# edantec/MPC_benchmark

Measured on AMD Instinct MI355X. Metric: mpc_solves_per_sec, higher is better.
Workload: dtype f64

## Files before the change

### mpc_benchmark_amd/csrc/legs.h

```cpp
#pragma once
#include "mfma_blocks.h"
#include "solver_kernels.h"

#define LEG_BARRIER() asm volatile("s_waitcnt lgkmcnt(0)\n\ts_barrier" ::: "memory")

#define LEG_LAUNDER() do { asm volatile("" : "+v"(tid), "+v"(lane)); wv = __builtin_amdgcn_readfirstlane(tid >> 6); } while (0)

#define LK_THREADS 512
#define LK_U 20
#define LK_PT 13
#define LK_TILES 5

struct LkLds {
  int np, mp, nzp, lda, ldp, ldm, nb, nbm;
  int AB, PR, TM, ZN, vec, total_bytes;
  unsigned mg_nzp, mg_np, mg_mp;
};
static inline constexpr LkLds make_lk_lds(int n, int m) {
  LkLds s{};
  s.np = (n + 15) & ~15; s.mp = (m + 15) & ~15; s.nzp = s.np + s.mp; s.lda = s.nzp + 1; s.ldp = s.np + 1; s.ldm = s.mp + 1;
  s.nb = s.np / 16; s.nbm = s.mp / 16;
  s.mg_nzp = magic_div(s.nzp); s.mg_np = magic_div(s.np); s.mg_mp = magic_div(s.mp);
  int o = 0;
  auto take = [&](int cnt) { int r = o; o += (cnt + 1) & ~1; return r; };
  const int pr = s.np * s.ldp > s.mp * s.np + s.mp * s.ldm ? s.np * s.ldp : s.mp * s.np + s.mp * s.ldm;
  s.AB = take(s.np * s.lda); s.PR = take(pr); s.TM = take(6 * s.nzp + 6 * s.np + 40); s.ZN = take(16 * s.ldm); s.vec = take(s.mp + 3 * s.np + 80 + 8);
  s.total_bytes = o * 8;
  return s;
}

template <int MP, int FN = 0, int FM = 0>
__global__ void __launch_bounds__(LK_THREADS) k_leg_knot(SolverArgs a, LkLds Srt, int chunk) {
  constexpr bool FX = FN > 0;
  constexpr LkLds SC_ = FX ? make_lk_lds(FN, FM) : LkLds{};
  LkLds S_ = Srt;
  if constexpr (FX) S_ = SC_;
  const LkLds& S = S_;
  constexpr int NAB = (80 * (80 + MP) + LK_THREADS - 1) / LK_THREADS, NK = (MP * 80 + LK_THREADS - 1) / LK_THREADS;
  constexpr int NMU = (MP * MP + LK_THREADS - 1) / LK_THREADS, NZN = (16 * MP + LK_THREADS - 1) / LK_THREADS;
  const Layout& L = a.L;
  const int b = blockIdx.y;
  int tid = threadIdx.x, lane = tid & 63;
  constexpr int nthr = LK_THREADS, nw = LK_THREADS / 64;
  int wv = __builtin_amdgcn_readfirstlane(tid >> 6);
  const InstState& st = a.inst[b];
  if (st.done || st.skip_step) return;
  const int n = FX ? FN : L.n, nz = FX ? FN + FM : L.nz, np = S.np, mp = S.mp, nzp = S.nzp, lda = S.lda, ldp = S.ldp, ldm = S.ldm, nb = S.nb, nbm = S.nbm;
  const int kbeg = blockIdx.x * chunk, kend = (kbeg + chunk < L.N) ? kbeg + chunk : L.N;
  const double mud = st.mu * a.opt.dyn_al_scale;
  extern __shared__ __attribute__((aligned(16))) double sm[];
  double *AB = sm + S.AB, *PR = sm + S.PR, *ZN = sm + S.ZN, *vec = sm + S.vec;
  double *KM = PR, *PT = PR, *U1 = PR, *MU = PR + mp * np;
  double *TMP = sm + S.TM, *PT6 = TMP + 6 * nzp, *c6 = PT6 + 6 * np;
  double *kf = vec, *y0 = vec + mp, *z0 = y0 + np, *t6 = z0 + np, *g6 = t6 + 36, *mxs = g6 + 36;
  int* cnt = (int*)(mxs + np);
  long long tk0_ = clock64();
#define LK_PROF(slot) do { if (a.prof && k == 1 && b == 1 && tid == 0) { const long long t1_ = clock64(); a.prof[64 + 32 + (slot)] += (double)(t1_ - tk0_); tk0_ = t1_; } } while (0)

  double pab[NAB], pkm[NK], ptv[LK_PT], pmu[NMU], pzn[NZN], psm = 0.0, pact = 0.0;
  auto request_ab = [&](int k) {
    const double* kn = knot_ptr(a, b, k);
    const double* g = gain_ptr(a, b, k);
    const int m = (int)kn[L.oMISC + MISC_M], c = (int)kn[L.oMISC + MISC_NC];
#pragma unroll
    for (int u = 0; u < NAB; ++u) {
      const int idx = tid + u * nthr, i = qdiv(idx, S.mg_nzp), zp = (idx - qdiv(idx, S.mg_nzp) * nzp);
      const int z = (zp < n) ? zp : ((zp >= np && zp - np < m) ? n + zp - np : -1);
      pab[u] = (idx < np * nzp && i < n && z >= 0) ? kn[L.oAB + (size_t)i * nz + z] : 0.0;
    }
#pragma unroll
    for (int u = 0; u < NK; ++u) {
      const int idx = tid + u * nthr, l = qdiv(idx, S.mg_np), j = (idx - qdiv(idx, S.mg_np) * np);
      pkm[u] = (idx < mp * np && l < m && j < n) ? g[L.oK + l * n + j] : 0.0;
    }
    psm = (tid < mp) ? ((tid < m) ? g[L.ok + tid] : 0.0) : ((tid >= 64 && tid < 100) ? g[L.oT6 + tid - 64] : ((tid >= 128 && tid < 128 + n) ? g[L.omx + tid - 128] : 0.0));
    pact = (tid < c) ? kn[L.oACT + tid] : 0.0;
  };
  auto request_pt = [&](int k) {
    const double* g = gain_ptr(a, b, k);
#pragma unroll
    for (int u = 0; u < LK_PT; ++u) {
      const int idx = tid + u * nthr, i = qdiv(idx, S.mg_np), j = (idx - qdiv(idx, S.mg_np) * np);
      ptv[u] = (idx < np * np && i < n && j < n) ? g[L.oMx + i * n + j] : 0.0;
    }
  };
  auto request_mu = [&](int k) {
    const double* g = gain_ptr(a, b, k);
#pragma unroll
    for (int u = 0; u < NMU; ++u) { const int idx = tid + u * nthr; pmu[u] = (idx < mp * mp) ? g[L.oMu + idx] : 0.0; }
#pragma unroll
// ... 160 lines not shown
            if (row < m && col < n) g[L.oKu + row * n + col] = -ures[sidx][q];
          }
        }
      }
#ifdef LK_SUBPROF
      LK_PROF(9);
#endif
      LEG_BARRIER();
      LK_PROF(5);
      for (int t = wv; t < nb * nb; t += nw) {
        const int ri = t / nb, cj = t % nb, col = cj * 16 + (lane & 15);
        double ptt[4];
#pragma unroll
        for (int q = 0; q < 4; ++q) {
          const int row = ri * 16 + (lane >> 4) + 4 * q;
          const bool in = row < n && col < n;
          ptt[q] = (in && row >= 6 && col >= 6) ? g[L.oMx + row * n + col] : 0.0;
        }
        d4_t acc = d4_t{0, 0, 0, 0};
        mma_tile<false>(acc, AB + (ri * 16) * lda + np, lda, 1, U1 + cj * 16, np, 1, mp, lane);
#pragma unroll
        for (int q = 0; q < 4; ++q) {
          const int row = ri * 16 + (lane >> 4) + 4 * q;
          if (row < n && col < n) {
            const double tt = (row < 6 && col < 6) ? g6[row * 6 + col] : (row == col ? 1.0 : 0.0);
            const double tp = (row < 6 && col < 6) ? c6[row * 6 + col] : (col < 6 ? PT6[row * 6 + col] : (row < 6 ? PT6[col * 6 + row] : ptt[q]));
            g[L.oGam + row * n + col] = -acc[q] - mud * (tt - mud * tp);
          }
        }
      }
      LK_PROF(6);
    } else if (par_next) request_mu(k + 1);
  }
}

struct LcLds { int np, ldp, nb; int LM, BA, BB, vec, total_bytes; unsigned mg_np, mg_ldp; };
static inline constexpr int lc_ld(int np) { int ld = np; while ((ld & 31) != 16) ++ld; return ld; }
static inline constexpr LcLds make_lc_lds(int n) {
  LcLds s{};
  s.np = (n + 15) & ~15; s.ldp = lc_ld(s.np); s.nb = s.np / 16;
  s.mg_np = magic_div(s.np); s.mg_ldp = magic_div(s.ldp);
  int o = 0;
  auto take = [&](int cnt) { int r = o; o += (cnt + 1) & ~1; return r; };
  s.LM = take(s.np * s.ldp); s.BA = take(s.np * s.ldp); s.BB = take(s.np * s.ldp); s.vec = take(3 * s.np + 16);
  s.total_bytes = o * 8;
  return s;
}
#define LC_TILES 4
#define LC_STILES 2

template <int FN = 0>
__global__ void __launch_bounds__(LK_THREADS) k_leg_condense(SolverArgs a, LcLds Srt) {
  constexpr bool FX = FN > 0;
  constexpr LcLds SC_ = FX ? make_lc_lds(FN) : LcLds{};
  LcLds S_ = Srt;
  if constexpr (FX) S_ = SC_;
  const LcLds& S = S_;
  const Layout& L = a.L;
  constexpr int nthr = LK_THREADS, nw = LK_THREADS / 64;
  const int j = blockIdx.x, b = blockIdx.y;
  int tid = threadIdx.x, lane = tid & 63, wv = __builtin_amdgcn_readfirstlane(tid >> 6);
  const InstState& st = a.inst[b];
  if (st.done || st.skip_step) return;
  const int n = FX ? FN : L.n, np = S.np, ldp = S.ldp, nb = S.nb;
  const int ks = leg_start(a, j), ke = leg_start(a, j + 1) - 1;
  extern __shared__ __attribute__((aligned(16))) double sm[];
  double *LM = sm + S.LM, *BA = sm + S.BA, *BB = sm + S.BB, *sg = sm + S.vec, *phi = sg + np;
  for (int idx = tid; idx < np * ldp; idx += nthr) { const int i = qdiv(idx, S.mg_ldp), c0 = (idx - qdiv(idx, S.mg_ldp) * ldp); LM[idx] = (i == c0 && i < n) ? 1.0 : 0.0; }
  for (int i = tid; i < np; i += nthr) sg[i] = 0.0;
  d4_t sacc[LC_STILES];
  int tri[LC_STILES], tcj[LC_STILES];
#pragma unroll
  for (int sidx = 0; sidx < LC_STILES; ++sidx) {
    sacc[sidx] = d4_t{0, 0, 0, 0};
    int ri = 0, rem = wv + sidx * nw;
    while (rem > ri) { rem -= ri + 1; ++ri; }
    tri[sidx] = ri; tcj[sidx] = rem;
  }
  const int nst = nb * (nb + 1) / 2;
  double pa[LK_PT], pb[LK_PT], pphi;
  auto prefetch = [&](int kk) {
    const double* gk = gain_ptr(a, b, kk);
#pragma unroll
    for (int u = 0; u < LK_PT; ++u) {
      const int idx = tid + u * nthr, i = qdiv(idx, S.mg_np), c0 = (idx - qdiv(idx, S.mg_np) * np);
      const bool ok = idx < np * np && i < n && c0 < n;
      const int src = ok ? i * n + c0 : 0;
      pa[u] = gk[L.oPhi + src] * (ok ? 1.0 : 0.0);
      pb[u] = gk[L.oGam + src] * (ok ? 1.0 : 0.0);
    }
    pphi = gk[L.ophi + (tid < n ? tid : 0)];
  };
  prefetch(ke);
// ... 48 lines not shown
    LC_PROF(5);
    LEG_BARRIER();
    LC_PROF(6);
    LEG_LAUNDER();
    double* gk = gain_ptr(a, b, k);
#pragma unroll
    for (int sidx = 0; sidx < LC_TILES; ++sidx) {
      const int t = wv + sidx * nw;
      if (t < nb * nb) {
        const int ri = t / nb, cj = t % nb, col = cj * 16 + (lane & 15);
        tile_store(LM + (ri * 16) * ldp + cj * 16, ldp, lres[sidx], lane);
#pragma unroll
        for (int q = 0; q < 4; ++q) { const int row = ri * 16 + (lane >> 4) + 4 * q; if (row < n && col < n) gk[L.oLm + row * n + col] = lres[sidx][q]; }
      }
    }
    LEG_BARRIER();
    LC_PROF(7);
  }
  double* lr = leg_ptr(a, b, j);
#pragma unroll
  for (int sidx = 0; sidx < LC_STILES; ++sidx)
    if (wv + sidx * nw < nst) {
      const int col = tcj[sidx] * 16 + (lane & 15);
#pragma unroll
      for (int q = 0; q < 4; ++q) {
        const int row = tri[sidx] * 16 + (lane >> 4) + 4 * q;
        if (row < n && col < n) {
          if (tri[sidx] != tcj[sidx]) { lr[L.lSg + row * n + col] = sacc[sidx][q]; lr[L.lSg + col * n + row] = sacc[sidx][q]; }
          else if (col <= row) { lr[L.lSg + row * n + col] = sacc[sidx][q]; lr[L.lSg + col * n + row] = sacc[sidx][q]; }
        }
      }
    }
  for (int i = tid; i < n; i += nthr) lr[L.lsg + i] = sg[i];
}

struct LxLds { int np, mp, ldp, nb, nbm; int PC, MA, RB, vec, iw, total_bytes; unsigned mg_np, mg_ldp; };
static inline constexpr LxLds make_lx_lds(int n, int m) {
  LxLds s{};
  s.np = (n + 15) & ~15; s.mp = (m + 15) & ~15; s.ldp = s.np + 1; s.nb = s.np / 16; s.nbm = s.mp / 16;
  s.mg_np = magic_div(s.np); s.mg_ldp = magic_div(s.ldp);
  int o = 0;
  auto take = [&](int cnt) { int r = o; o += (cnt + 1) & ~1; return r; };
  s.PC = take(s.np * s.ldp); s.MA = take(s.np * s.ldp); s.RB = take(s.np * s.ldp);
  s.vec = take(8 * s.np + 16 + 128);
  s.iw = o;
  s.total_bytes = o * 8 + (2 * s.np + 8) * 4;
  return s;
}

template <bool TR>
DEV void leg_load_mat(double* dst, int ldp, int np, const double* src, int n, int tid, int nthr, unsigned mg_np) {
  const struct { unsigned mg_np; } S = {mg_np};
  double v[LK_PT];
#pragma unroll
  for (int u = 0; u < LK_PT; ++u) {
    const int idx = tid + u * nthr, i = qdiv(idx, S.mg_np), c0 = (idx - qdiv(idx, S.mg_np) * np);
    const bool ok = idx < np * np && i < n && c0 < n;
    v[u] = src[ok ? i * n + c0 : 0] * (ok ? 1.0 : 0.0);
  }
#pragma unroll
  for (int u = 0; u < LK_PT; ++u) {
    const int idx = tid + u * nthr, i = qdiv(idx, S.mg_np), c0 = (idx - qdiv(idx, S.mg_np) * np);
    if (idx < np * np) dst[TR ? c0 * ldp + i : i * ldp + c0] = v[u];
  }
}

// ... 380 lines not shown
```

### mpc_benchmark_amd/csrc/mpc_hip.hip

```cpp
#include <hip/hip_runtime.h>
#include <mutex>
#include <map>
#include <cmath>
#include <cstdio>
#include <cstdlib>
#include <cstring>
#include <limits>
#include <stdexcept>
#include <string>
#include <utility>
#include <vector>

#include "eval_multibody_host.h"
#include "eval_reuse_kernels.h"
#include "eval_vector.h"
#include "riccati_mfma.h"
#include "closed_loop.h"
#include "legs.h"
#include "legs_tree.h"
#include "pipeline_glue.h"
#include "pipeline_ikid_glue.h"
#include "pipeline_contacts.h"
#include "pipeline_fd_glue.h"
#include "sim_record.h"
// ... 122 lines not shown
  bool refine_now = false;
  SimPlant plant;
  std::vector<uint8_t> slot_dirty;
  bool dirty_all = false;
  bool spec_skip_pass = false;
  unsigned long long dirty_now[MPC_DIRTY_WORDS] = {};
  static constexpr int PATCH_RING = 4;
  char* patch_pin[PATCH_RING] = {};
  size_t patch_cap[PATCH_RING] = {};
  hipEvent_t patch_ev[PATCH_RING] = {};
  int patch_next = 0;
  char* d_patch = nullptr;
  size_t d_patch_cap = 0;
  double* h_xnext[2] = {nullptr, nullptr};
  std::vector<double> leg_mu;
  static constexpr int ASYNC_DEPTH = 2;
  InstState* h_status[ASYNC_DEPTH] = {nullptr, nullptr};
  hipEvent_t status_ev[ASYNC_DEPTH] = {nullptr, nullptr};
  int async_head = 0, async_pending = 0;
  static constexpr int STAGE_RING = 8;
  char* stage_pin[STAGE_RING] = {};
  hipEvent_t stage_ev[STAGE_RING] = {};
  int stage_next = 0;
  RicLds ric{};
  int ric_fixed = 0;
  ClLds cl{};
  bool use_mfma_riccati = false;
  LkLds lk{};
  LcLds lc{};
  LxLds lx{};
  bool legs_ok = false;
  bool env_chain = false, env_plain = false, env_reject_failed = false;
  int env_tree_sweeps = 0, env_trace = -1;
  double* d_legbuf = nullptr;
  double* d_treebuf = nullptr;
  int leg_cap = 0;
  TreeDesc tree{};
  bool use_tree() const {
    return eff_legs() >= 3 && d_treebuf != nullptr && !env_chain;
  }
  bool leg_guess_valid = false;
  int leg_guess_now = 0;
  int eff_legs() const {
    if (!legs_ok) return 1;
    int J = opt.riccati_legs;
    if (J > MPC_MAX_LEGS) J = MPC_MAX_LEGS;
    if (J > L.N) J = L.N;
    return J < 1 ? 1 : J;
  }
  struct ProfSlot {
    const char* name;
    std::vector<std::pair<hipEvent_t, hipEvent_t>> ev;
    size_t used = 0;
  };
  bool profiling = false;
  unsigned prof_mask = ~0u;
  std::vector<ProfSlot> prof;

  template <class F> void timed(int slot, const char* name, F&& launch) {
    if (!profiling || !((prof_mask >> slot) & 1u) || pass_is_corrector) { launch(); return; }
    if ((int)prof.size() <= slot) prof.resize(slot + 1);
    ProfSlot& p = prof[slot];
    p.name = name;
    if (p.used == p.ev.size()) {
      hipEvent_t e0, e1;
      HIP_OK(hipEventCreate(&e0));
// ... 47 lines not shown
  HIP_OK(hipStreamSynchronize(s->stream));
}

static void ensure_leg_capacity(mpc_solver* s, int legs) {
  const Layout& L = s->L;
  int need = legs < 1 ? 1 : legs;
  if (need >= 3 && need < 4) need = 4;
  if (need <= s->leg_cap) return;
  HIP_OK(hipStreamSynchronize(s->stream));
  auto regrow = [&](double*& p, size_t count) {
    if (p) HIP_OK(hipFree(p));
    p = nullptr;
    HIP_OK(hipMalloc((void**)&p, (count ? count : 1) * sizeof(double)));
    HIP_OK(hipMemsetAsync(p, 0, (count ? count : 1) * sizeof(double), s->stream));
  };
  const size_t B = L.B;
  regrow(s->d_work, B * need * (size_t)L.work_stride);
  if (s->legs_ok) {
    regrow(s->d_legbuf, B * (size_t)(need > 1 ? need - 1 : 1) * L.leg_stride);
    regrow(s->d_treebuf, B * (size_t)need * L.tree_stride);
  }
  s->leg_cap = need;
  s->leg_guess_valid = false;
  HIP_OK(hipStreamSynchronize(s->stream));
}

static void create_impl(mpc_solver* s, const mpc_dims& d) {
  s->dims = d;
  { const char* e;
    e = getenv("MPC_LEGS_CHAIN"); s->env_chain = e && atoi(e) > 0;
    e = getenv("MPC_LEGS_PLAIN"); s->env_plain = e && atoi(e) > 0;
    e = getenv("MPC_HIP_REJECT_FAILED"); s->env_reject_failed = e && atoi(e) > 0;
    e = getenv("MPC_TREE_SWEEPS"); s->env_tree_sweeps = e ? atoi(e) : 0;
    e = getenv("MPC_HIP_TRACE"); s->env_trace = e ? atoi(e) : -1; }
  HIP_OK(hipSetDevice(d.device));
  {
    static int created = 0;
    const char* pe = getenv("MPC_HIP_STREAM_PRIO");
    if (pe && atoi(pe) > 0) {
      int lo = 0, hi = 0;
      HIP_OK(hipDeviceGetStreamPriorityRange(&lo, &hi));
      const int levels = lo - hi + 1;
      const int prio = hi + (created++ % levels);
      HIP_OK(hipStreamCreateWithPriority(&s->stream, hipStreamNonBlocking, prio));
      if (atoi(pe) > 1) fprintf(stderr, "[mpc] stream priority %d (range %d..%d)\n", prio, hi, lo);
    } else {
      HIP_OK(hipStreamCreateWithFlags(&s->stream, hipStreamNonBlocking));
    }
  }
  Layout& L = s->L;
  L.N = d.horizon; L.B = d.batch; L.space = d.space; L.nx = d.nx; L.n = d.ndx; L.m = d.nu; L.c = d.nc_max > 0 ? d.nc_max : 1;
  L.nj = 0;
  L.max_stage_ints = d.max_stage_ints; L.max_stage_doubles = d.max_stage_doubles;
  L.n_alpha = 8;
  make_layout(L);
  Layout& T = s->LT;
  T = L;
  {
    int o = 0;
    auto take = [&](int cnt) { int r = o; o += align2(cnt); return r; };
    T.oCV = take(L.c); T.oCT = take(L.c); T.oLO = take(L.c); T.oHI = take(L.c); T.oDT = take(L.c); T.oACT = take(L.c);
    T.oF = take(L.n); T.oMISC = take(MISC_COUNT);
    T.oH = T.oG = T.oAB = T.oE6 = T.oT6k = T.oD12 = T.oCD = T.oXD = T.oWR = T.oXN = 0;
    T.knot_stride = o;
  }
  if (s->riccati_lds() > 160 * 1024) throw std::runtime_error("problem dimensions exceed the LDS budget of the Riccati kernel");
  const size_t B = d.batch, N1 = d.horizon + 1, N = d.horizon;
  s->d_stage_desc = s->alloc<int32_t>(N1 * L.max_stage_ints);
// ... 32 lines not shown
    if (c3.total_bytes > 160 * 1024) c3 = make_ric_lds(L.n, L.m, L.c, 3, 0);
    if (c3.total_bytes <= 160 * 1024 && c3.ovl && (c3.st_lds || c3.mp * c3.np <= L.n * L.nz)) s->ric = c3;
  }
  if (s->ric.total_bytes > 160 * 1024 && ((L.n + 15) & ~15) * ((L.m + 15) & ~15) <= L.n * L.n) {
    s->ric = make_ric_lds(L.n, L.m, L.c, 2);
    if (s->ric.total_bytes > 160 * 1024) s->ric = make_ric_lds(L.n, L.m, L.c, 2, 0);
  }
  if (s->ric.total_bytes > 160 * 1024) s->ric = make_ric_lds(L.n, L.m, L.c, 0);
  if (s->ric.total_bytes > 160 * 1024) s->ric = make_ric_lds(L.n, L.m, L.c, 0, 0);
  if (sq_ok && s->ric.gfull) { s->ric.sq = 1; s->ric.nv = L.n / 2; }
  s->cl = make_cl_lds(L.n, L.m);
  if (s->cl.total_bytes <= 160 * 1024)
    lds_attr_max((const void*)k_closed_loop, s->cl.total_bytes);
  s->use_mfma_riccati = s->ric.total_bytes <= 160 * 1024 && (s->ric.st_lds || s->ric.mp * s->ric.np <= L.n * L.nz) && !getenv("MPC_HIP_GENERIC_RICCATI");
  if (s->use_mfma_riccati)
  {
    lds_attr_max((const void*)k_riccati_mfma<RIC_THREADS, 96>, s->ric.total_bytes);
    lds_attr_max((const void*)k_riccati_mfma<RIC_THREADS, 80>, s->ric.total_bytes);
    lds_attr_max((const void*)k_riccati_mfma<RIC_THREADS, 96, true>, s->ric.total_bytes);
    lds_attr_max((const void*)k_riccati_mfma<RIC_THREADS, 80, true>, s->ric.total_bytes);
    lds_attr_max((const void*)k_riccati_mfma<RIC_SMALL_THREADS, 16>, s->ric.total_bytes);
  }
  s->lk = make_lk_lds(L.n, L.m); s->lc = make_lc_lds(L.n); s->lx = make_lx_lds(L.n, L.m);
  s->legs_ok = s->use_mfma_riccati && s->ric.np <= 80 && s->ric.mp <= 48 && L.c <= 256 && s->ric.gfull >= 1 && s->lk.total_bytes <= 160 * 1024 &&
               s->lc.total_bytes <= 160 * 1024 && s->lx.total_bytes <= 160 * 1024 && !getenv("MPC_HIP_NO_LEGS");
  if (s->legs_ok) {
    lds_attr_max((const void*)k_riccati_mfma<RIC_THREADS, 80, true, true>, s->ric.total_bytes);
    s->ric_fixed = 0;
    if (!getenv("MPC_HIP_GENERIC_DIMS") && s->ric.sq) {
#define X(ID, FN, FM, GF, ST, NPV, MPV) if (!s->ric_fixed && L.n == FN && L.m == FM && L.nz == FN + FM && ric_same_layout(s->ric, ric_fixed_layout(FN, FM, true, GF, ST))) s->ric_fixed = ID;
      MPC_FIXED_MODELS(X)
#undef X
    }
#define X(ID, FN, FM, GF, ST, NPV, MPV) if (s->ric_fixed == ID) { \
      lds_attr_max((const void*)k_riccati_mfma<RIC_THREADS, 80, true, true, FN, FM, GF, ST>, s->ric.total_bytes); \
      lds_attr_max((const void*)k_leg_knot<MPV, FN, FM>, s->lk.total_bytes); \
      lds_attr_max((const void*)k_leg_condense<FN>, s->lc.total_bytes); \
      lds_attr_max((const void*)k_leg_compose<NPV, FN, FM>, s->lx.total_bytes); \
      lds_attr_max((const void*)k_leg_tree_down<NPV, FN, FM>, s->lx.total_bytes); }
    MPC_FIXED_MODELS(X)
#undef X
    lds_attr_max((const void*)k_riccati_mfma<RIC_THREADS, 80, false, true>, s->ric.total_bytes);
    lds_attr_max((const void*)k_riccati_mfma<RIC_SMALL_THREADS, 16, false, true>, s->ric.total_bytes);
    lds_attr_max((const void*)k_leg_knot<16>, s->lk.total_bytes);
    lds_attr_max((const void*)k_leg_knot<32>, s->lk.total_bytes);
    lds_attr_max((const void*)k_leg_knot<48>, s->lk.total_bytes);
    lds_attr_max((const void*)k_leg_condense<0>, s->lc.total_bytes);
    lds_attr_max((const void*)k_leg_consensus<16>, s->lx.total_bytes);
    lds_attr_max((const void*)k_leg_consensus<32>, s->lx.total_bytes);
    lds_attr_max((const void*)k_leg_consensus<48>, s->lx.total_bytes);
    lds_attr_max((const void*)k_leg_consensus<64>, s->lx.total_bytes);
    lds_attr_max((const void*)k_leg_consensus<80>, s->lx.total_bytes);
    lds_attr_max((const void*)k_leg_compose<16>, s->lx.total_bytes);
    lds_attr_max((const void*)k_leg_compose<32>, s->lx.total_bytes);
    lds_attr_max((const void*)k_leg_compose<48>, s->lx.total_bytes);
    lds_attr_max((const void*)k_leg_compose<64>, s->lx.total_bytes);
    lds_attr_max((const void*)k_leg_compose<80>, s->lx.total_bytes);
    lds_attr_max((const void*)k_leg_tree_down<16>, s->lx.total_bytes);
    lds_attr_max((const void*)k_leg_tree_down<32>, s->lx.total_bytes);
    lds_attr_max((const void*)k_leg_tree_down<48>, s->lx.total_bytes);
    lds_attr_max((const void*)k_leg_tree_down<64>, s->lx.total_bytes);
    lds_attr_max((const void*)k_leg_tree_down<80>, s->lx.total_bytes);
  }
  ensure_leg_capacity(s, s->eff_legs());
  HIP_OK(hipStreamSynchronize(s->stream));
}

__global__ void __launch_bounds__(256) k_bcast_params(double* inst, const double* shared, int slot, int nslots, int stride) {
  const int b = blockIdx.y;
  const double* src = shared + (size_t)slot * stride;
  double* dst = inst + ((size_t)b * nslots + slot) * stride;
  for (int i = blockIdx.x * 256 + threadIdx.x; i < stride; i += gridDim.x * 256) dst[i] = src[i];
}
static void bcast_slot_to_instances(mpc_solver* s, int slot) {
  if (!s->d_inst_params) return;
  const Layout& L = s->L;
  hipLaunchKernelGGL(k_bcast_params, dim3(4, L.B), dim3(256), 0, s->stream, s->d_inst_params, s->d_stage_params, slot, L.N + 1, L.max_stage_doubles);
  for (int b = 0; b < L.B; ++b)
    std::memcpy(s->h_inst_params.data() + ((size_t)b * (L.N + 1) + slot) * L.max_stage_doubles, s->h_params.data() + (size_t)slot * L.max_stage_doubles,
                (size_t)L.max_stage_doubles * sizeof(double));
// ... 156 lines not shown
  const Layout& L = s->L;
  SolverArgs a = s->args();
  if (ncand <= 0) return;
  if (L.space == MPC_SPACE_VECTOR) {
    if (!trial) hipLaunchKernelGGL(k_eval_vector<0>, dim3(a.only_knot >= 0 ? 1 : L.N + 1, L.B, 1), dim3(64), 0, s->stream, a, s->L, s->d_knots, 0);
    else hipLaunchKernelGGL(k_eval_vector<1>, dim3(L.N + 1, L.B, ncand), dim3(64), 0, s->stream, a, s->LT, s->d_tknots, cand0);
  } else {
    launch_eval_multibody(s->stream, a, s->LT, (trial && !with_derivs) ? s->d_tknots : s->d_knots, s->d_mbwork, s->mb_work_stride, trial, cand0, ncand, 0, 0.0, with_derivs, nullptr, s->contact_dyn);
  }
  HIP_OK(hipGetLastError());
}

static void launch_pass(mpc_solver* s) {
  const Layout& L = s->L;
  if (s->pass_in_run > 0 && s->tick_reuse && s->opt.max_iters <= 4) {
    s->reuse_this_pass = true; s->reuse_same_now = true;
    for (int w = 0; w < MPC_DIRTY_WORDS; ++w) s->dirty_now[w] = 0ull;
  }
  SolverArgs a = s->args();
  if (a.spec_next) hipLaunchKernelGGL(k_copy_spec, dim3(32, L.B), dim3(256), 0, s->stream, a);
  s->timed(0, "k_eval_stage", [&] { launch_eval(s, false); });
  if (a.reuse_on) hipLaunchKernelGGL(k_reproject, dim3(L.N + 1, L.B), dim3(256), 0, s->stream, a);
  s->reuse_this_pass = false; s->reuse_same_now = false;
  s->spec_next_now = false;
  s->timed(1, "k_lagrangian", [&] { hipLaunchKernelGGL(k_lagrangian, dim3(L.N + 1, L.B), dim3(64), 0, s->stream, a); });
  s->timed(2, "k_decide", [&] { hipLaunchKernelGGL(k_decide, dim3(L.B), dim3(128), 0, s->stream, a); });
  a.abdz = nullptr;
  const int J = a.nlegs;
  const bool plain = s->env_plain;
  const bool tree = s->use_tree();
  if (tree && s->tree.J != J) s->tree = make_tree_desc(J);
  int sweeps = (J > 1 && !plain && !s->leg_guess_valid) ? (tree ? s->tree.nlev + 1 : 2) : 1;
  if (tree && !plain && s->env_tree_sweeps > sweeps) sweeps = s->env_tree_sweeps;
  for (int sweep = 0; sweep < sweeps; ++sweep) {
  s->leg_guess_now = (J > 1 && !plain && (s->leg_guess_valid || sweep > 0)) ? 1 : 0;
  a = s->args();
  a.abdz = nullptr;
  s->timed(3, "k_riccati_backward", [&] {
    if (J > 1) {
      if (s->ric.np == 16 && s->ric.mp == 16 && L.c <= RIC_SMALL_THREADS)
        hipLaunchKernelGGL(HIP_KERNEL_NAME(k_riccati_mfma<RIC_SMALL_THREADS, 16, false, true>), dim3(L.B * J), dim3(RIC_SMALL_THREADS), s->ric.total_bytes, s->stream, a, s->ric);
#define X(ID, FN, FM, GF, ST, NPV, MPV) else if (s->ric_fixed == ID) hipLaunchKernelGGL(HIP_KERNEL_NAME(k_riccati_mfma<RIC_THREADS, 80, true, true, FN, FM, GF, ST>), dim3(L.B * J), dim3(RIC_THREADS), s->ric.total_bytes, s->stream, a, s->ric);
      MPC_FIXED_MODELS(X)
#undef X
      else if (s->ric.sq) hipLaunchKernelGGL(HIP_KERNEL_NAME(k_riccati_mfma<RIC_THREADS, 80, true, true>), dim3(L.B * J), dim3(RIC_THREADS), s->ric.total_bytes, s->stream, a, s->ric);
      else hipLaunchKernelGGL(HIP_KERNEL_NAME(k_riccati_mfma<RIC_THREADS, 80, false, true>), dim3(L.B * J), dim3(RIC_THREADS), s->ric.total_bytes, s->stream, a, s->ric);
    }
    else if (s->use_mfma_riccati && s->ric.np == 16 && s->ric.mp == 16 && L.c <= RIC_SMALL_THREADS)
      hipLaunchKernelGGL(HIP_KERNEL_NAME(k_riccati_mfma<RIC_SMALL_THREADS, 16>), dim3(L.B), dim3(RIC_SMALL_THREADS), s->ric.total_bytes, s->stream, a, s->ric);
    else if (s->use_mfma_riccati && s->ric.sq && s->ric.np <= 80) hipLaunchKernelGGL(HIP_KERNEL_NAME(k_riccati_mfma<RIC_THREADS, 80, true>), dim3(L.B), dim3(RIC_THREADS), s->ric.total_bytes, s->stream, a, s->ric);
    else if (s->use_mfma_riccati && s->ric.sq) hipLaunchKernelGGL(HIP_KERNEL_NAME(k_riccati_mfma<RIC_THREADS, 96, true>), dim3(L.B), dim3(RIC_THREADS), s->ric.total_bytes, s->stream, a, s->ric);
    else if (s->use_mfma_riccati && s->ric.np <= 80) hipLaunchKernelGGL(HIP_KERNEL_NAME(k_riccati_mfma<RIC_THREADS, 80>), dim3(L.B), dim3(RIC_THREADS), s->ric.total_bytes, s->stream, a, s->ric);
    else if (s->use_mfma_riccati) hipLaunchKernelGGL(HIP_KERNEL_NAME(k_riccati_mfma<RIC_THREADS, 96>), dim3(L.B), dim3(RIC_THREADS), s->ric.total_bytes, s->stream, a, s->ric);
    else hipLaunchKernelGGL(k_riccati_backward, dim3(L.B), dim3(256), s->riccati_lds(), s->stream, a);
  });
  if (J > 1) {
    s->timed(12, "k_closed_loop", [&] {
      static const int chunk_env = getenv("MPC_LEG_KNOT_CHUNK") ? atoi(getenv("MPC_LEG_KNOT_CHUNK")) : 0;
      const int chunk = chunk_env > 0 ? chunk_env : 1;
      const dim3 grid((L.N + chunk - 1) / chunk, L.B);
      if (false) {}
#define X(ID, FN, FM, GF, ST, NPV, MPV) else if (s->ric_fixed == ID) hipLaunchKernelGGL((k_leg_knot<MPV, FN, FM>), grid, dim3(LK_THREADS), s->lk.total_bytes, s->stream, a, s->lk, chunk);
      MPC_FIXED_MODELS(X)
#undef X
      else if (s->lk.mp <= 16) hipLaunchKernelGGL(k_leg_knot<16>, grid, dim3(LK_THREADS), s->lk.total_bytes, s->stream, a, s->lk, chunk);
      else if (s->lk.mp <= 32) hipLaunchKernelGGL(k_leg_knot<32>, grid, dim3(LK_THREADS), s->lk.total_bytes, s->stream, a, s->lk, chunk);
      else hipLaunchKernelGGL(k_leg_knot<48>, grid, dim3(LK_THREADS), s->lk.total_bytes, s->stream, a, s->lk, chunk);
    });
    s->timed(13, "k_leg_condense", [&] {
      if (false) {}
#define X(ID, FN, FM, GF, ST, NPV, MPV) else if (s->ric_fixed == ID) hipLaunchKernelGGL(k_leg_condense<FN>, dim3(J - 1, L.B), dim3(LK_THREADS), s->lc.total_bytes, s->stream, a, s->lc);
      MPC_FIXED_MODELS(X)
#undef X
      else hipLaunchKernelGGL(k_leg_condense<0>, dim3(J - 1, L.B), dim3(LK_THREADS), s->lc.total_bytes, s->stream, a, s->lc);
    });
    if (tree) s->timed(14, "k_leg_consensus", [&] {
      const TreeDesc& T = s->tree;
#define MPC_TREE_LAUNCH(NPV) do { \
        for (int lev = 0; lev < T.nlev; ++lev) hipLaunchKernelGGL(k_leg_compose<NPV>, dim3(T.lev_cnt[lev] + 1, L.B, 2), dim3(LCMP_THREADS), s->lx.total_bytes, s->stream, a, s->lx, T, lev); } while (0)
      if (false) {
#define X(ID, FN, FM, GF, ST, NPV, MPV) } else if (s->ric_fixed == ID) { for (int lev = 0; lev < T.nlev; ++lev) hipLaunchKernelGGL((k_leg_compose<NPV, FN, FM>), dim3(T.lev_cnt[lev] + 1, L.B, 2), dim3(LCMP_THREADS), s->lx.total_bytes, s->stream, a, s->lx, T, lev);
      MPC_FIXED_MODELS(X)
#undef X
      } else switch (s->lx.np) {
        case 16: MPC_TREE_LAUNCH(16); break;
        case 32: MPC_TREE_LAUNCH(32); break;
        case 48: MPC_TREE_LAUNCH(48); break;
        case 64: MPC_TREE_LAUNCH(64); break;
        default: MPC_TREE_LAUNCH(80); break;
      }
#undef MPC_TREE_LAUNCH
    });
    if (tree) s->timed(16, "k_leg_tree_down", [&] {
      const TreeDesc& T = s->tree;
      if (false) {
#define X(ID, FN, FM, GF, ST, NPV, MPV) } else if (s->ric_fixed == ID) { for (int lev = T.nlev - 1; lev >= 0; --lev) hipLaunchKernelGGL((k_leg_tree_down<NPV, FN, FM>), dim3(T.lev_cnt[lev] + (lev == T.nlev - 1 ? 1 : 0), L.B), dim3(LK_THREADS), s->lx.total_bytes, s->stream, a, s->lx, T, lev);
      MPC_FIXED_MODELS(X)
#undef X
      } else switch (s->lx.np) {
        case 16: for (int lev = T.nlev - 1; lev >= 0; --lev) hipLaunchKernelGGL(k_leg_tree_down<16>, dim3(T.lev_cnt[lev] + (lev == T.nlev - 1 ? 1 : 0), L.B), dim3(LK_THREADS), s->lx.total_bytes, s->stream, a, s->lx, T, lev); break;
        case 32: for (int lev = T.nlev - 1; lev >= 0; --lev) hipLaunchKernelGGL(k_leg_tree_down<32>, dim3(T.lev_cnt[lev] + (lev == T.nlev - 1 ? 1 : 0), L.B), dim3(LK_THREADS), s->lx.total_bytes, s->stream, a, s->lx, T, lev); break;
        case 48: for (int lev = T.nlev - 1; lev >= 0; --lev) hipLaunchKernelGGL(k_leg_tree_down<48>, dim3(T.lev_cnt[lev] + (lev == T.nlev - 1 ? 1 : 0), L.B), dim3(LK_THREADS), s->lx.total_bytes, s->stream, a, s->lx, T, lev); break;
// ... 424 lines not shown
    else if (mode == 3 || mode == 4) s->phase_timers = (mode == 3);
    else if (mode >= 16) { s->profiling = true; s->prof_mask = (unsigned)mode >> 4; }
    else { s->profiling = (mode != 0); s->prof_mask = ~0u; }
  })
}

int mpc_kernel_info(mpc_solver* s, int32_t idx, char* name, int32_t name_cap, int32_t* info) {
  if (!s) return -2;
  try {
    HIP_OK(hipSetDevice(s->dims.device));
    const Layout& L = s->L;
    struct Ent { const char* name; const void* fn; int block; int dyn; long long grid; };
    std::vector<Ent> e;
    const int J = s->eff_legs();
    if (L.space == MPC_SPACE_VECTOR) {
      e.push_back({"k_eval_vector<0> (stage kernel, value + derivatives)", (const void*)k_eval_vector<0>, 64, 0, (long long)(L.N + 1) * L.B});
      e.push_back({"k_eval_vector<1> (linesearch candidate)", (const void*)k_eval_vector<1>, 64, 0, (long long)(L.N + 1) * L.B});
    } else {
      const MbLds ml = make_mb_lds(L.nj, L.n / 2, L.nx - L.n / 2, L.m, L.nz, s->contact_dyn);
      e.push_back({"k_eval_multibody<0> (stage kernel, value + derivatives)", eval_multibody_kernel(0), EVAL_THREADS, ml.total_bytes, (long long)(L.N + 1) * L.B});
      e.push_back({"k_eval_multibody<3> (alpha = 1 candidate with derivatives)", eval_multibody_kernel(3), EVAL_THREADS, ml.total_bytes, (long long)(L.N + 1) * L.B});
      e.push_back({"k_eval_multibody<1> (backtracking candidates, values only)", eval_multibody_kernel(1), EVAL_THREADS, ml.total_bytes, (long long)(L.N + 1) * L.B});
    }
    const bool small = s->ric.np == 16 && s->ric.mp == 16 && L.c <= RIC_SMALL_THREADS;
    if (J > 1) {
      if (small) e.push_back({"k_riccati_mfma<256,16,false,true> (sweep, legs)", (const void*)k_riccati_mfma<RIC_SMALL_THREADS, 16, false, true>, RIC_SMALL_THREADS, s->ric.total_bytes, (long long)L.B * J});
#define X(ID, FN, FM, GF, ST, NPV, MPV) else if (s->ric_fixed == ID) e.push_back({"k_riccati_mfma<512,80,true,true," #FN "," #FM "," #GF "," #ST "> (sweep, legs, fixed dimensions)", (const void*)k_riccati_mfma<RIC_THREADS, 80, true, true, FN, FM, GF, ST>, RIC_THREADS, s->ric.total_bytes, (long long)L.B * J});
      MPC_FIXED_MODELS(X)
#undef X
      else if (s->ric.sq) e.push_back({"k_riccati_mfma<512,80,true,true> (sweep, legs)", (const void*)k_riccati_mfma<RIC_THREADS, 80, true, true>, RIC_THREADS, s->ric.total_bytes, (long long)L.B * J});
      else e.push_back({"k_riccati_mfma<512,80,false,true> (sweep, legs)", (const void*)k_riccati_mfma<RIC_THREADS, 80, false, true>, RIC_THREADS, s->ric.total_bytes, (long long)L.B * J});
      const void* lk = s->lk.mp <= 16 ? (const void*)k_leg_knot<16> : (s->lk.mp <= 32 ? (const void*)k_leg_knot<32> : (const void*)k_leg_knot<48>);
      const void* lcd = (const void*)k_leg_condense<0>;
      const char *lk_name = "k_leg_knot", *lcd_name = "k_leg_condense", *lcmp_name = "k_leg_compose (first level of the tree over the cuts)", *ltd_name = "k_leg_tree_down (last level)";
      const void *lcmp_fixed = nullptr, *ltd_fixed = nullptr;
#define X(ID, FN, FM, GF, ST, NPV, MPV) if (s->ric_fixed == ID) { lk = (const void*)k_leg_knot<MPV, FN, FM>; lcd = (const void*)k_leg_condense<FN>; lcmp_fixed = (const void*)k_leg_compose<NPV, FN, FM>; ltd_fixed = (const void*)k_leg_tree_down<NPV, FN, FM>; \
        lk_name = "k_leg_knot<" #MPV "," #FN "," #FM "> (fixed dimensions)"; lcd_name = "k_leg_condense<" #FN "> (fixed dimensions)"; \
        lcmp_name = "k_leg_compose<" #NPV "," #FN "," #FM "> (first level of the tree over the cuts, fixed dimensions)"; ltd_name = "k_leg_tree_down<" #NPV "," #FN "," #FM "> (last level, fixed dimensions)"; }
      MPC_FIXED_MODELS(X)
#undef X
      e.push_back({lk_name, lk, LK_THREADS, s->lk.total_bytes, (long long)L.N * L.B});
      e.push_back({lcd_name, lcd, LK_THREADS, s->lc.total_bytes, (long long)(J - 1) * L.B});
      if (s->use_tree()) {
        const TreeDesc T = make_tree_desc(J);
        const void* lc = s->lx.np == 16 ? (const void*)k_leg_compose<16> : s->lx.np == 32 ? (const void*)k_leg_compose<32> : s->lx.np == 48 ? (const void*)k_leg_compose<48>
                       : s->lx.np == 64 ? (const void*)k_leg_compose<64> : (const void*)k_leg_compose<80>;
        const void* ld = s->lx.np == 16 ? (const void*)k_leg_tree_down<16> : s->lx.np == 32 ? (const void*)k_leg_tree_down<32> : s->lx.np == 48 ? (const void*)k_leg_tree_down<48>
                       : s->lx.np == 64 ? (const void*)k_leg_tree_down<64> : (const void*)k_leg_tree_down<80>;
        e.push_back({lcmp_name, lcmp_fixed ? lcmp_fixed : lc, LCMP_THREADS, s->lx.total_bytes, (long long)(T.lev_cnt[0] + 1) * L.B * 2});
        e.push_back({ltd_name, ltd_fixed ? ltd_fixed : ld, LK_THREADS, s->lx.total_bytes, (long long)T.lev_cnt[0] * L.B});
      } else {
      const void* lx = s->lx.np == 16 ? (const void*)k_leg_consensus<16> : s->lx.np == 32 ? (const void*)k_leg_consensus<32> : s->lx.np == 48 ? (const void*)k_leg_consensus<48>
                     : s->lx.np == 64 ? (const void*)k_leg_consensus<64> : (const void*)k_leg_consensus<80>;
      e.push_back({"k_leg_consensus", lx, LK_THREADS, s->lx.total_bytes, (long long)L.B});
      }
      e.push_back({"k_leg_apply", (const void*)k_leg_apply, 256, 0, (long long)L.N * L.B});
      e.push_back({"k_forward_phi (forward sweeps of the legs)", L.m <= 32 ? (const void*)k_forward_phi<4, 10> : (const void*)k_forward_phi<6, 10>, 512, (int)(2 * L.n * sizeof(double)), (long long)L.B * J});
    } else if (s->use_mfma_riccati) {
      const void* fn = small ? (const void*)k_riccati_mfma<RIC_SMALL_THREADS, 16> : (s->ric.sq && s->ric.np <= 80) ? (const void*)k_riccati_mfma<RIC_THREADS, 80, true>
                     : s->ric.sq ? (const void*)k_riccati_mfma<RIC_THREADS, 96, true> : s->ric.np <= 80 ? (const void*)k_riccati_mfma<RIC_THREADS, 80> : (const void*)k_riccati_mfma<RIC_THREADS, 96>;
      e.push_back({"k_riccati_mfma (serial sweep)", fn, small ? RIC_SMALL_THREADS : RIC_THREADS, s->ric.total_bytes, (long long)L.B});
    } else e.push_back({"k_riccati_backward (serial sweep, no matrix cores)", (const void*)k_riccati_backward, 256, (int)s->riccati_lds(), (long long)L.B});
    e.push_back({"k_duals", (const void*)k_duals, 256, (int)((L.nz + 3 * L.n + 16 + 3 * L.c) * sizeof(double)), (long long)(L.N + 1) * L.B});
    e.push_back({"k_lagrangian", (const void*)k_lagrangian, 64, 0, (long long)(L.N + 1) * L.B});
    if (idx < 0 || idx >= (int)e.size()) return (int)e.size();
    const Ent& k = e[idx];
    hipFuncAttributes at;
    HIP_OK(hipFuncGetAttributes(&at, k.fn));
    int nb = 0;
    HIP_OK(hipOccupancyMaxActiveBlocksPerMultiprocessor(&nb, k.fn, k.block, (size_t)k.dyn));
    if (name && name_cap > 0) { strncpy(name, k.name, name_cap - 1); name[name_cap - 1] = 0; }
    info[0] = k.block; info[1] = at.numRegs; info[2] = (int)at.localSizeBytes; info[3] = (int)at.sharedSizeBytes; info[4] = k.dyn; info[5] = nb;
    info[6] = (int)k.grid; info[7] = nb * ((k.block + 63) / 64) / 4;
    return (int)e.size();
  } catch (const std::exception& ex) { s->err = ex.what(); return -1; }
// ... 384 lines not shown
    else if (nm == "K") mat(g.data() + L.oK, m, n, n);
    else if (nm == "kff") mat(g.data() + L.ok, 1, m, m);
    else if (nm == "Knu") { for (int i = 0; i < c; ++i) if (kn[L.oACT + i] == 0.0) for (int z = 0; z < n; ++z) g[L.oKnu + i * n + z] = 0.0; mat(g.data() + L.oKnu, c, n, n); }
    else if (nm == "knu") mat(g.data() + L.oknu, 1, c, c);
    else if (nm == "Mx") mat(g.data() + L.oMx, k < L.N ? n : 0, n, n);
    else if (nm == "mx") mat(g.data() + L.omx, 1, k < L.N ? n : 0, n);
    else if (nm == "Phi") mat(g.data() + L.oPhi, k < L.N ? n : 0, n, n);
    else if (nm == "phi") mat(g.data() + L.ophi, 1, k < L.N ? n : 0, n);
    else if (nm == "Gam") mat(g.data() + L.oGam, n, n, n);
    else if (nm == "Ku") mat(g.data() + L.oKu, m, n, n);
    else if (nm == "Lm") mat(g.data() + L.oLm, n, n, n);
    else if (nm == "Mu") mat(g.data() + L.oMu, m, m, L.mpad);
    else if (nm == "Znu" || nm == "Knup") {
      const bool zn = nm == "Znu";
      const int cols = zn ? m : n, ld = zn ? L.mpad : n;
      v.assign((size_t)c * cols, 0.0);
      int ai = 0;
      for (int i = 0; i < c; ++i) if (kn[L.oACT + i] != 0.0) { for (int j = 0; j < cols; ++j) v[(size_t)i * cols + j] = g[(zn ? L.oZnu : L.oKnup) + ai * ld + j]; ++ai; }
    }
    else if (nm == "Sg" || nm == "sg" || nm == "Zx" || nm == "zc" || nm == "calP" || nm == "calp" || nm == "theta") {
      if (!s->d_legbuf || k >= s->leg_cap - 1) throw std::runtime_error("debug_get: no such leg record");
      const double* lr = s->d_legbuf + ((size_t)b * (s->leg_cap - 1) + k) * L.leg_stride;
      if (nm == "Sg") dev_vec(lr + L.lSg, n * n); else if (nm == "sg") dev_vec(lr + L.lsg, n); else if (nm == "Zx") dev_vec(lr + L.lZx, n * n);
      else if (nm == "zc") dev_vec(lr + L.lzc, n); else if (nm == "calP") dev_vec(lr + L.ldP, n * n);
      else if (nm == "calp") dev_vec(lr + L.lcp, n);
      else dev_vec(lr + L.lth, n);
    }
    else if (nm == "ls_knot") {
      std::vector<double> tp((size_t)L.n_alpha * (L.N + 1));
      copy_sync(s, tp.data(), s->d_trial_phi + (size_t)b * L.n_alpha * (L.N + 1), tp.size() * sizeof(double), hipMemcpyDeviceToHost);
      for (int i = 0; i < L.n_alpha; ++i) v.push_back(tp[(size_t)i * (L.N + 1) + k]);
      v.push_back(kn[L.oMISC + MISC_COST]); v.push_back(kn[L.oMISC + MISC_PEN]);
    }
    else if (nm == "fixed_dims") v = {(double)s->ric_fixed};
    else if (nm == "ric_prof") { dev_vec(s->d_prof + (size_t)b * 64, 64); HIP_OK(hipMemsetAsync(s->d_prof + (size_t)b * 64, 0, 64 * sizeof(double), s->stream)); HIP_OK(hipStreamSynchronize(s->stream)); }
    else if (nm == "dx") dev_vec(s->d_dxs + ((size_t)b * (L.N + 1) + k) * n, n);
    else if (nm == "du") { if (k >= L.N) throw std::runtime_error("no du at the terminal knot"); dev_vec(s->d_dus + ((size_t)b * L.N + k) * L.m, L.m); }
    else if (nm == "dvs") dev_vec(s->d_dvs + ((size_t)b * (L.N + 1) + k) * L.c, L.c);
    else if (nm == "dlams") dev_vec(s->d_dlams + ((size_t)b * (L.N + 1) + k) * n, n);
    else throw std::runtime_error("debug_get: unknown quantity " + nm);
    if ((int)v.size() > cap) throw std::runtime_error("debug_get: output buffer too small");
    if (!v.empty()) std::memcpy(out, v.data(), v.size() * sizeof(double));
    return (int)v.size();
  } catch (const std::exception& e) {
    s->err = e.what();
    return -1;
  }
}

}

#include "walk_poses.h"
#include "walk_commands.h"
#include "sim_host.h"
#include "pipeline_loops.h"
```

Baseline: 11960.

## Fuse last leg's knot work into the condense kernel to fill idle CUs

Splits the leg knot and condense kernels into device bodies, then adds a combined kernel. In it the blocks for the first J-1 legs run condensation while the final block per batch processes the last leg's tail knots, which are dropped from the knot launch. The knot launch gets shorter and the tail work overlaps with condensation on CUs that would otherwise sit idle. It runs only when J*B fits in the CU count and N*B exceeds it. It risks higher LDS per block (max of both layouts) and a longer critical path if the tail block is slow.

```diff
diff --git a/mpc_benchmark_amd/csrc/legs.h b/mpc_benchmark_amd/csrc/legs.h
--- a/mpc_benchmark_amd/csrc/legs.h
+++ b/mpc_benchmark_amd/csrc/legs.h
@@ -30,7 +30,7 @@
 }
 
 template <int MP, int FN = 0, int FM = 0>
-__global__ void __launch_bounds__(LK_THREADS) k_leg_knot(SolverArgs a, LkLds Srt, int chunk) {
+DEV void leg_knot_body(const SolverArgs& a, const LkLds& Srt, const int b, const int kbeg, const int kend, const int prof_b, const int prof_k) {
   constexpr bool FX = FN > 0;
   constexpr LkLds SC_ = FX ? make_lk_lds(FN, FM) : LkLds{};
   LkLds S_ = Srt;
@@ -39,14 +39,12 @@
   constexpr int NAB = (80 * (80 + MP) + LK_THREADS - 1) / LK_THREADS, NK = (MP * 80 + LK_THREADS - 1) / LK_THREADS;
   constexpr int NMU = (MP * MP + LK_THREADS - 1) / LK_THREADS, NZN = (16 * MP + LK_THREADS - 1) / LK_THREADS;
   const Layout& L = a.L;
-  const int b = blockIdx.y;
   int tid = threadIdx.x, lane = tid & 63;
   constexpr int nthr = LK_THREADS, nw = LK_THREADS / 64;
   int wv = __builtin_amdgcn_readfirstlane(tid >> 6);
   const InstState& st = a.inst[b];
   if (st.done || st.skip_step) return;
   const int n = FX ? FN : L.n, nz = FX ? FN + FM : L.nz, np = S.np, mp = S.mp, nzp = S.nzp, lda = S.lda, ldp = S.ldp, ldm = S.ldm, nb = S.nb, nbm = S.nbm;
-  const int kbeg = blockIdx.x * chunk, kend = (kbeg + chunk < L.N) ? kbeg + chunk : L.N;
   const double mud = st.mu * a.opt.dyn_al_scale;
   extern __shared__ __attribute__((aligned(16))) double sm[];
   double *AB = sm + S.AB, *PR = sm + S.PR, *ZN = sm + S.ZN, *vec = sm + S.vec;
@@ -55,7 +53,7 @@
   double *kf = vec, *y0 = vec + mp, *z0 = y0 + np, *t6 = z0 + np, *g6 = t6 + 36, *mxs = g6 + 36;
   int* cnt = (int*)(mxs + np);
   long long tk0_ = clock64();
-#define LK_PROF(slot) do { if (a.prof && k == 1 && b == 1 && tid == 0) { const long long t1_ = clock64(); a.prof[64 + 32 + (slot)] += (double)(t1_ - tk0_); tk0_ = t1_; } } while (0)
+#define LK_PROF(slot) do { if (a.prof && k == prof_k && b == prof_b && tid == 0) { const long long t1_ = clock64(); a.prof[prof_b * 64 + 32 + (slot)] += (double)(t1_ - tk0_); tk0_ = t1_; } } while (0)
 
   double pab[NAB], pkm[NK], ptv[LK_PT], pmu[NMU], pzn[NZN], psm = 0.0, pact = 0.0;
   auto request_ab = [&](int k) {
@@ -282,6 +280,12 @@
       LK_PROF(6);
     } else if (par_next) request_mu(k + 1);
   }
+}
+
+template <int MP, int FN = 0, int FM = 0>
+__global__ void __launch_bounds__(LK_THREADS) k_leg_knot(SolverArgs a, LkLds Srt, int chunk, int kmax) {
+  const int kbeg = blockIdx.x * chunk, kend = (kbeg + chunk < kmax) ? kbeg + chunk : kmax;
+  if (kbeg < kend) leg_knot_body<MP, FN, FM>(a, Srt, blockIdx.y, kbeg, kend, 1, 1);
 }
 
 struct LcLds { int np, ldp, nb; int LM, BA, BB, vec, total_bytes; unsigned mg_np, mg_ldp; };
@@ -300,7 +304,7 @@
 #define LC_STILES 2
 
 template <int FN = 0>
-__global__ void __launch_bounds__(LK_THREADS) k_leg_condense(SolverArgs a, LcLds Srt) {
+DEV void leg_condense_body(const SolverArgs& a, const LcLds& Srt, const int j, const int b) {
   constexpr bool FX = FN > 0;
   constexpr LcLds SC_ = FX ? make_lc_lds(FN) : LcLds{};
   LcLds S_ = Srt;
@@ -308,7 +312,6 @@
   const LcLds& S = S_;
   const Layout& L = a.L;
   constexpr int nthr = LK_THREADS, nw = LK_THREADS / 64;
-  const int j = blockIdx.x, b = blockIdx.y;
   int tid = threadIdx.x, lane = tid & 63, wv = __builtin_amdgcn_readfirstlane(tid >> 6);
   const InstState& st = a.inst[b];
   if (st.done || st.skip_step) return;
@@ -423,6 +426,21 @@
       }
     }
   for (int i = tid; i < n; i += nthr) lr[L.lsg + i] = sg[i];
+}
+
+template <int FN = 0>
+__global__ void __launch_bounds__(LK_THREADS) k_leg_condense(SolverArgs a, LcLds Srt) {
+  leg_condense_body<FN>(a, Srt, blockIdx.x, blockIdx.y);
+}
+
+template <int MP, int FN = 0, int FM = 0>
+__global__ void __launch_bounds__(LK_THREADS) k_leg_condense_tail(SolverArgs a, LcLds Sc, LkLds Sk, int tail) {
+  const int j = blockIdx.x, b = blockIdx.y;
+  if (j + 1 < a.nlegs) leg_condense_body<FN>(a, Sc, j, b);
+  else {
+    const int kend = a.L.N, kbeg = kend - tail;
+    if (kbeg >= 0 && kbeg < kend) leg_knot_body<MP, FN, FM>(a, Sk, b, kbeg, kend, -1, -1);
+  }
 }
 
 struct LxLds { int np, mp, ldp, nb, nbm; int PC, MA, RB, vec, iw, total_bytes; unsigned mg_np, mg_ldp; };
diff --git a/mpc_benchmark_amd/csrc/mpc_hip.hip b/mpc_benchmark_amd/csrc/mpc_hip.hip
--- a/mpc_benchmark_amd/csrc/mpc_hip.hip
+++ b/mpc_benchmark_amd/csrc/mpc_hip.hip
@@ -178,6 +178,18 @@
   bool legs_ok = false;
   bool env_chain = false, env_plain = false, env_reject_failed = false;
   int env_tree_sweeps = 0, env_trace = -1;
+  int env_tail_knots = -1, cu_count = 0;
+  int tail_last = 0, tail_sweeps_last = 0;
+  long long tail_fused = 0, tail_separate = 0;
+  long long leg_passes_multi = 0, leg_passes_single = 0;
+  int leg_tail_knots(int J) const {
+    if (J < 2 || env_tail_knots == 0) return 0;
+    const int last = L.N - (int)((long long)(J - 1) * L.N / J);
+    if (env_tail_knots > 0) return env_tail_knots < last ? env_tail_knots : last;
+    if ((long long)J * L.B > cu_count || (long long)L.N * L.B <= cu_count) return 0;
+    const int t = 21 * (L.N / J) / 25;
+    return t < last ? t : last;
+  }
   double* d_legbuf = nullptr;
   double* d_treebuf = nullptr;
   int leg_cap = 0;
@@ -291,8 +303,11 @@
     e = getenv("MPC_LEGS_PLAIN"); s->env_plain = e && atoi(e) > 0;
     e = getenv("MPC_HIP_REJECT_FAILED"); s->env_reject_failed = e && atoi(e) > 0;
     e = getenv("MPC_TREE_SWEEPS"); s->env_tree_sweeps = e ? atoi(e) : 0;
-    e = getenv("MPC_HIP_TRACE"); s->env_trace = e ? atoi(e) : -1; }
+    e = getenv("MPC_HIP_TRACE"); s->env_trace = e ? atoi(e) : -1;
+    e = getenv("MPC_LEG_TAIL_KNOTS"); s->env_tail_knots = e ? (atoi(e) > 0 ? atoi(e) : 0) : -1; }
   HIP_OK(hipSetDevice(d.device));
+  HIP_OK(hipDeviceGetAttribute(&s->cu_count, hipDeviceAttributeMultiprocessorCount, d.device));
+  { const char* e = getenv("MPC_LEG_TAIL_CUS"); if (e && atoi(e) > 0) s->cu_count = atoi(e); }
   {
     static int created = 0;
     const char* pe = getenv("MPC_HIP_STREAM_PRIO");
@@ -391,10 +406,12 @@
       MPC_FIXED_MODELS(X)
 #undef X
     }
+    const int leg_tail_lds = s->lc.total_bytes > s->lk.total_bytes ? s->lc.total_bytes : s->lk.total_bytes;
 #define X(ID, FN, FM, GF, ST, NPV, MPV) if (s->ric_fixed == ID) { \
       lds_attr_max((const void*)k_riccati_mfma<RIC_THREADS, 80, true, true, FN, FM, GF, ST>, s->ric.total_bytes); \
       lds_attr_max((const void*)k_leg_knot<MPV, FN, FM>, s->lk.total_bytes); \
       lds_attr_max((const void*)k_leg_condense<FN>, s->lc.total_bytes); \
+      lds_attr_max((const void*)k_leg_condense_tail<MPV, FN, FM>, leg_tail_lds); \
       lds_attr_max((const void*)k_leg_compose<NPV, FN, FM>, s->lx.total_bytes); \
       lds_attr_max((const void*)k_leg_tree_down<NPV, FN, FM>, s->lx.total_bytes); }
     MPC_FIXED_MODELS(X)
@@ -405,6 +422,9 @@
     lds_attr_max((const void*)k_leg_knot<32>, s->lk.total_bytes);
     lds_attr_max((const void*)k_leg_knot<48>, s->lk.total_bytes);
     lds_attr_max((const void*)k_leg_condense<0>, s->lc.total_bytes);
+    lds_attr_max((const void*)k_leg_condense_tail<16>, leg_tail_lds);
+    lds_attr_max((const void*)k_leg_condense_tail<32>, leg_tail_lds);
+    lds_attr_max((const void*)k_leg_condense_tail<48>, leg_tail_lds);
     lds_attr_max((const void*)k_leg_consensus<16>, s->lx.total_bytes);
     lds_attr_max((const void*)k_leg_consensus<32>, s->lx.total_bytes);
     lds_attr_max((const void*)k_leg_consensus<48>, s->lx.total_bytes);
@@ -627,6 +647,9 @@
   if (tree && s->tree.J != J) s->tree = make_tree_desc(J);
   int sweeps = (J > 1 && !plain && !s->leg_guess_valid) ? (tree ? s->tree.nlev + 1 : 2) : 1;
   if (tree && !plain && s->env_tree_sweeps > sweeps) sweeps = s->env_tree_sweeps;
+  const int tail = s->leg_tail_knots(J);
+  s->tail_last = tail; s->tail_sweeps_last = sweeps;
+  if (J > 1) { if (sweeps > 1) s->leg_passes_multi++; else s->leg_passes_single++; }
   for (int sweep = 0; sweep < sweeps; ++sweep) {
   s->leg_guess_now = (J > 1 && !plain && (s->leg_guess_valid || sweep > 0)) ? 1 : 0;
   a = s->args();
@@ -653,16 +676,30 @@
     s->timed(12, "k_closed_loop", [&] {
       static const int chunk_env = getenv("MPC_LEG_KNOT_CHUNK") ? atoi(getenv("MPC_LEG_KNOT_CHUNK")) : 0;
       const int chunk = chunk_env > 0 ? chunk_env : 1;
-      const dim3 grid((L.N + chunk - 1) / chunk, L.B);
+      const int kmax = L.N - tail;
+      const dim3 grid((kmax + chunk - 1) / chunk, L.B);
       if (false) {}
-#define X(ID, FN, FM, GF, ST, NPV, MPV) else if (s->ric_fixed == ID) hipLaunchKernelGGL((k_leg_knot<MPV, FN, FM>), grid, dim3(LK_THREADS), s->lk.total_bytes, s->stream, a, s->lk, chunk);
+#define X(ID, FN, FM, GF, ST, NPV, MPV) else if (s->ric_fixed == ID) hipLaunchKernelGGL((k_leg_knot<MPV, FN, FM>), grid, dim3(LK_THREADS), s->lk.total_bytes, s->stream, a, s->lk, chunk, kmax);
       MPC_FIXED_MODELS(X)
 #undef X
-      else if (s->lk.mp <= 16) hipLaunchKernelGGL(k_leg_knot<16>, grid, dim3(LK_THREADS), s->lk.total_bytes, s->stream, a, s->lk, chunk);
-      else if (s->lk.mp <= 32) hipLaunchKernelGGL(k_leg_knot<32>, grid, dim3(LK_THREADS), s->lk.total_bytes, s->stream, a, s->lk, chunk);
-      else hipLaunchKernelGGL(k_leg_knot<48>, grid, dim3(LK_THREADS), s->lk.total_bytes, s->stream, a, s->lk, chunk);
+      else if (s->lk.mp <= 16) hipLaunchKernelGGL(k_leg_knot<16>, grid, dim3(LK_THREADS), s->lk.total_bytes, s->stream, a, s->lk, chunk, kmax);
+      else if (s->lk.mp <= 32) hipLaunchKernelGGL(k_leg_knot<32>, grid, dim3(LK_THREADS), s->lk.total_bytes, s->stream, a, s->lk, chunk, kmax);
+      else hipLaunchKernelGGL(k_leg_knot<48>, grid, dim3(LK_THREADS), s->lk.total_bytes, s->stream, a, s->lk, chunk, kmax);
     });
-    s->timed(13, "k_leg_condense", [&] {
+    if (tail > 0) s->timed(13, "k_leg_condense", [&] {
+      const int lds = s->lc.total_bytes > s->lk.total_bytes ? s->lc.total_bytes : s->lk.total_bytes;
+      const dim3 grid(J, L.B);
+      s->tail_fused++;
+      if (false) {}
+#define X(ID, FN, FM, GF, ST, NPV, MPV) else if (s->ric_fixed == ID) hipLaunchKernelGGL((k_leg_condense_tail<MPV, FN, FM>), grid, dim3(LK_THREADS), lds, s->stream, a, s->lc, s->lk, tail);
+      MPC_FIXED_MODELS(X)
+#undef X
+      else if (s->lk.mp <= 16) hipLaunchKernelGGL(k_leg_condense_tail<16>, grid, dim3(LK_THREADS), lds, s->stream, a, s->lc, s->lk, tail);
+      else if (s->lk.mp <= 32) hipLaunchKernelGGL(k_leg_condense_tail<32>, grid, dim3(LK_THREADS), lds, s->stream, a, s->lc, s->lk, tail);
+      else hipLaunchKernelGGL(k_leg_condense_tail<48>, grid, dim3(LK_THREADS), lds, s->stream, a, s->lc, s->lk, tail);
+    });
+    else s->timed(13, "k_leg_condense", [&] {
+      s->tail_separate++;
       if (false) {}
 #define X(ID, FN, FM, GF, ST, NPV, MPV) else if (s->ric_fixed == ID) hipLaunchKernelGGL(k_leg_condense<FN>, dim3(J - 1, L.B), dim3(LK_THREADS), s->lc.total_bytes, s->stream, a, s->lc);
       MPC_FIXED_MODELS(X)
@@ -1153,15 +1190,19 @@
       else e.push_back({"k_riccati_mfma<512,80,false,true> (sweep, legs)", (const void*)k_riccati_mfma<RIC_THREADS, 80, false, true>, RIC_THREADS, s->ric.total_bytes, (long long)L.B * J});
       const void* lk = s->lk.mp <= 16 ? (const void*)k_leg_knot<16> : (s->lk.mp <= 32 ? (const void*)k_leg_knot<32> : (const void*)k_leg_knot<48>);
       const void* lcd = (const void*)k_leg_condense<0>;
+      const void* lct = s->lk.mp <= 16 ? (const void*)k_leg_condense_tail<16> : (s->lk.mp <= 32 ? (const void*)k_leg_condense_tail<32> : (const void*)k_leg_condense_tail<48>);
+      const char* lct_name = "k_leg_condense_tail (condensation + the last leg's knots)";
       const char *lk_name = "k_leg_knot", *lcd_name = "k_leg_condense", *lcmp_name = "k_leg_compose (first level of the tree over the cuts)", *ltd_name = "k_leg_tree_down (last level)";
       const void *lcmp_fixed = nullptr, *ltd_fixed = nullptr;
-#define X(ID, FN, FM, GF, ST, NPV, MPV) if (s->ric_fixed == ID) { lk = (const void*)k_leg_knot<MPV, FN, FM>; lcd = (const void*)k_leg_condense<FN>; lcmp_fixed = (const void*)k_leg_compose<NPV, FN, FM>; ltd_fixed = (const void*)k_leg_tree_down<NPV, FN, FM>; \
+#define X(ID, FN, FM, GF, ST, NPV, MPV) if (s->ric_fixed == ID) { lk = (const void*)k_leg_knot<MPV, FN, FM>; lcd = (const void*)k_leg_condense<FN>; lct = (const void*)k_leg_condense_tail<MPV, FN, FM>; lct_name = "k_leg_condense_tail<" #MPV "," #FN "," #FM "> (fixed dimensions)"; lcmp_fixed = (const void*)k_leg_compose<NPV, FN, FM>; ltd_fixed = (const void*)k_leg_tree_down<NPV, FN, FM>; \
         lk_name = "k_leg_knot<" #MPV "," #FN "," #FM "> (fixed dimensions)"; lcd_name = "k_leg_condense<" #FN "> (fixed dimensions)"; \
         lcmp_name = "k_leg_compose<" #NPV "," #FN "," #FM "> (first level of the tree over the cuts, fixed dimensions)"; ltd_name = "k_leg_tree_down<" #NPV "," #FN "," #FM "> (last level, fixed dimensions)"; }
       MPC_FIXED_MODELS(X)
 #undef X
-      e.push_back({lk_name, lk, LK_THREADS, s->lk.total_bytes, (long long)L.N * L.B});
-      e.push_back({lcd_name, lcd, LK_THREADS, s->lc.total_bytes, (long long)(J - 1) * L.B});
+      const int tail = s->leg_tail_knots(J);
+      e.push_back({lk_name, lk, LK_THREADS, s->lk.total_bytes, (long long)(L.N - tail) * L.B});
+      if (tail > 0) e.push_back({lct_name, lct, LK_THREADS, s->lc.total_bytes > s->lk.total_bytes ? s->lc.total_bytes : s->lk.total_bytes, (long long)J * L.B});
+      else e.push_back({lcd_name, lcd, LK_THREADS, s->lc.total_bytes, (long long)(J - 1) * L.B});
       if (s->use_tree()) {
         const TreeDesc T = make_tree_desc(J);
         const void* lc = s->lx.np == 16 ? (const void*)k_leg_compose<16> : s->lx.np == 32 ? (const void*)k_leg_compose<32> : s->lx.np == 48 ? (const void*)k_leg_compose<48>
@@ -1612,6 +1653,8 @@
       for (int i = 0; i < L.n_alpha; ++i) v.push_back(tp[(size_t)i * (L.N + 1) + k]);
       v.push_back(kn[L.oMISC + MISC_COST]); v.push_back(kn[L.oMISC + MISC_PEN]);
     }
+    else if (nm == "leg_tail") v = {(double)s->tail_last, (double)s->tail_fused, (double)s->tail_separate, (double)s->tail_sweeps_last, (double)s->eff_legs(), (double)s->cu_count,
+                                   (double)s->leg_passes_multi, (double)s->leg_passes_single};
     else if (nm == "fixed_dims") v = {(double)s->ric_fixed};
     else if (nm == "ric_prof") { dev_vec(s->d_prof + (size_t)b * 64, 64); HIP_OK(hipMemsetAsync(s->d_prof + (size_t)b * 64, 0, 64 * sizeof(double), s->stream)); HIP_OK(hipStreamSynchronize(s->stream)); }
     else if (nm == "dx") dev_vec(s->d_dxs + ((size_t)b * (L.N + 1) + k) * n, n);
```

After: 12170, median of 6. +1.8%, better.
